# zhouhuan2005/deep-fusion

Measured on AMD Instinct MI355X. Metric: fused conv3x3+relu+conv1x1 int8 images/sec, higher is better.
Workload: dtype u8*s8->s32 (int8 MFMA), f32 requant, s32 out

## Files before the change

deep-fusion_amd/csrc/conv_mfma.cuh:

```cuda
#pragma once

#include <type_traits>

#include "dfx_device.cuh"

namespace dfx {

constexpr int MFMA_THREADS = 1024;
constexpr int MFMA_TEAMS = 2;
constexpr int MFMA_CW = 7;
constexpr int MFMA_NB = 4;
#ifndef DFX_STAMPS
constexpr int MFMA_CTRL_BYTES = 128;
#else
constexpr int MFMA_CTRL_BYTES = 128 + 16 * 8 * 4;
#endif
constexpr int MFMA_LC = 22;
constexpr int MFMA_SPIN_LIMIT = 1 << 24;

constexpr int MAGIC0_BITS = 0x4B400000;
constexpr float MAGIC0_F = 12582912.0f;
constexpr int MAGIC1_BITS = 0x3E22F983;
constexpr int MAGIC1_LO = -0x22F983;
constexpr int MAGIC1_HI = 0x7FFFFF - 0x22F983;

__host__ __device__ constexpr int mfma_cst_floats(int oc, int oc1) { return oc1 ? 3 * oc + 5 * oc1 : 5 * oc; }

constexpr int CTL_NEXT = 0;
constexpr int CTL_END = 1;
constexpr int CTL_FULL = 4;
constexpr int CTL_DONE = 8;
constexpr int CTL_INFO = 16;

__device__ __forceinline__ v16i mfma_i8(v4i a, v4i b, v16i c) {
  return __builtin_amdgcn_mfma_i32_32x32x32_i8(a, b, c, 0, 0, 0);
}

template <int CP>
__device__ __forceinline__ int chunk_swizzle(int X) {
  if (CP == 2) return (X >> 3) & 1;
  if (CP == 4) return (X >> 2) & 3;
  return (X >> 1) & 7;
}

struct MfmaGeom {
  int th, tw;
  int uy, ux;
  int linear;
  int total_units;
  int row_chunks;
  int tile_chunks;
  unsigned row_magic;
  unsigned tw_magic;
  unsigned upi_magic, ux_magic;
  int ntu;
  unsigned ntu_magic;
  int claim_limit;
  int mode0, mode1;
  int s0_uniform;
  float s0_value;
  int tile_stride;
  int static_rounds;
  int pool;
  int lazy_queue;
  int half_from;
  int *queue;
#ifdef DFX_STAMPS
  unsigned long long *prof;
#endif
#ifdef DFX_TRACE
  int *trace;
#endif
};

#ifdef DFX_TRACE
#define DFX_TRACE_AT(code, v0, v1)                                                                      \
  do {                                                                                                  \
    if ((int)threadIdx.x == __builtin_amdgcn_readfirstlane((int)threadIdx.x)) {  \
      int *tr_ = g.trace + ((size_t)blockIdx.x * 16 + (threadIdx.x >> 6)) * 4;                          \
      __hip_atomic_fetch_add(tr_ + 3, 1, __ATOMIC_RELAXED, __HIP_MEMORY_SCOPE_SYSTEM);  \
      if ((threadIdx.x & 63) != 0 && tr_[1] == 0)    \
        __hip_atomic_store(tr_ + 1, (int)(code), __ATOMIC_RELAXED, __HIP_MEMORY_SCOPE_SYSTEM);           \
      (void)(v0);                                                                                       \
      __hip_atomic_store(tr_ + 2, (int)__builtin_amdgcn_read_exec_lo(), __ATOMIC_RELAXED, __HIP_MEMORY_SCOPE_SYSTEM); (void)(v1); \
      __hip_atomic_store(tr_ + 0, (int)(code), __ATOMIC_RELEASE, __HIP_MEMORY_SCOPE_SYSTEM);            \
    }                                                                                                   \
  } while (0)
#else
#define DFX_TRACE_AT(code, v0, v1)
#endif

#ifdef DFX_STAMPS
__device__ __forceinline__ unsigned long long dfx_stamp() {
  unsigned long long t;
  __builtin_amdgcn_sched_barrier(0);
  asm volatile("s_memtime %0\n\ts_waitcnt lgkmcnt(0)" : "=s"(t)::"memory");
  __builtin_amdgcn_sched_barrier(0);
  return t;
}
#define DFX_STAMP(var) const unsigned long long var = dfx_stamp()
#define DFX_ACC(slot, expr) prof_acc[slot] += (expr)
#define DFX_TLOG(n, v0, v1, v2, v3)                                                                      \
  do {                                                                                                   \
    if ((n) < 8) {                                                                                       \
      unsigned long long *tl_ = g.prof + (size_t)gridDim.x * 256 +                                       \
                                (((size_t)blockIdx.x * 16 + (threadIdx.x >> 6)) * 8 + (n)) * 4;          \
      tl_[0] = (v0); tl_[1] = (v1); tl_[2] = (v2); tl_[3] = (v3);                                        \
    }                                                                                                    \
  } while (0)
#define DFX_LACC(slot, expr)                                                                             \
  __hip_atomic_fetch_add(ctrl + 32 + 8 * (int)(threadIdx.x >> 6) + (slot), (int)(unsigned)(expr), __ATOMIC_RELAXED, \
                         __HIP_MEMORY_SCOPE_WORKGROUP)
#else
#define DFX_STAMP(var)
#define DFX_ACC(slot, expr)
#define DFX_LACC(slot, expr)
#define DFX_TLOG(n, v0, v1, v2, v3)
#endif
// ... 281 lines not shown
      hrow = (v & 1) * hth;
    }
    n = g.upi_magic ? (int)__umulhi((unsigned)unit, g.upi_magic) : unit;
    const int u = unit - n * upi;
    uyi = g.ux_magic ? (int)__umulhi((unsigned)u, g.ux_magic) : u;
    uxi = u - uyi * g.ux;
  };
  auto unit_origin = [&](int unit, const uint8_t *&src_n, int &y0, int &x0) {
    int n, uyi, uxi, hrow, hth;
    unit_split(unit, n, uyi, uxi, hrow, hth);
    y0 = uyi * g.th + hrow - a.pt;
    x0 = uxi * g.tw - a.pl;
    src_n = a.src + (size_t)n * a.ih * a.iw * IC;
  };

  auto unit_info = [&](int unit, int &pix0, int &thtw, int &tprm) {
    int n, uyi, uxi, hrow, hth;
    unit_split(unit, n, uyi, uxi, hrow, hth);
    const int y0 = uyi * g.th + hrow, x0 = uxi * g.tw;
    const int th = max(0, min(hth, a.oh - y0)), tw = min(g.tw, a.ow - x0);
    const int tpr = g.pool ? (tw + 15) >> 4 : (tw + 31) >> 5;
    pix0 = g.pool ? (n * (a.oh >> 1) + (y0 >> 1)) * (a.ow >> 1) + (x0 >> 1)
                  : (n * a.oh + y0) * a.ow + x0;
    thtw = (th << 16) | tw;
    tprm = tpr > 1 ? (int)(((1ull << 32) + tpr - 1) / tpr) : 0;
  };

  const int wg = (gridDim.x % 8 == 0) ? (int)(blockIdx.x % 8) * (int)(gridDim.x / 8) + (int)(blockIdx.x / 8)
                                      : (int)blockIdx.x;
  auto stream_id = [&](int tm) { return tm * (int)gridDim.x + wg; };
  const bool coop0 = g.static_rounds >= 1;

  auto ctl_load = [&](int idx) {
    return __builtin_amdgcn_readfirstlane(
        __hip_atomic_load(ctrl + idx, __ATOMIC_ACQUIRE, __HIP_MEMORY_SCOPE_WORKGROUP));
  };
  auto ctl_store = [&](int idx, int v) {
    __hip_atomic_store(ctrl + idx, v, __ATOMIC_RELEASE, __HIP_MEMORY_SCOPE_WORKGROUP);
  };

  auto stage_weights = [&]() {
    constexpr int NT = MFMA_TEAMS * MFMA_CW * 64;
    constexpr int TT = MFMA_CW * 64;
    const int ctid = (team * MFMA_CW + cw) * 64 + lane, tctid = cw * 64 + lane;
    const v4i *s = reinterpret_cast<const v4i *>(a.wei);
    v4i *d = reinterpret_cast<v4i *>(w0s);
    const int total = OCB * 9 * ICB * 64 + NCB * OCB * 64 + (mfma_cst_floats(OC, OC1) * 4 + 15) / 16;
    unsigned char *slot = tiles + (size_t)team * g.tile_stride;
    const int unit0 = stream_id(team);
    const bool tile0 = coop0 && unit0 < g.total_units;
    const uint8_t *src_n = a.src;
    int y0 = 0, x0 = 0;
    if (tile0) unit_origin(unit0, src_n, y0, x0);
    for (int base = 0; base < total; base += 4 * NT) {
      const int q0 = base + ctid, last = total - 1;
      const v4i t0 = s[min(q0 + 0 * NT, last)];
      const v4i t1 = s[min(q0 + 1 * NT, last)];
      const v4i t2 = s[min(q0 + 2 * NT, last)];
      const v4i t3 = s[min(q0 + 3 * NT, last)];
      v4i u0 = x80, u1 = x80, u2 = x80, u3 = x80;
      if (tile0 && base == 0) {
        u0 = load_granule(src_n, y0, x0, min(tctid + 0 * TT, g.tile_chunks - 1));
        u1 = load_granule(src_n, y0, x0, min(tctid + 1 * TT, g.tile_chunks - 1));
        u2 = load_granule(src_n, y0, x0, min(tctid + 2 * TT, g.tile_chunks - 1));
        u3 = load_granule(src_n, y0, x0, min(tctid + 3 * TT, g.tile_chunks - 1));
      }
      d[min(q0 + 0 * NT, last)] = t0;
      d[min(q0 + 1 * NT, last)] = t1;
      d[min(q0 + 2 * NT, last)] = t2;
      d[min(q0 + 3 * NT, last)] = t3;
      if (tile0 && base == 0) {
        if (tctid + 0 * TT < g.tile_chunks) *reinterpret_cast<v4i *>(slot + 16 * (tctid + 0 * TT)) = u0;
        if (tctid + 1 * TT < g.tile_chunks) *reinterpret_cast<v4i *>(slot + 16 * (tctid + 1 * TT)) = u1;
        if (tctid + 2 * TT < g.tile_chunks) *reinterpret_cast<v4i *>(slot + 16 * (tctid + 2 * TT)) = u2;
        if (tctid + 3 * TT < g.tile_chunks) *reinterpret_cast<v4i *>(slot + 16 * (tctid + 3 * TT)) = u3;
      }
    }
    if (tile0) {
      for (int base = 4 * TT; base < g.tile_chunks; base += 4 * TT) {
        const int q0 = base + tctid;
        const v4i t0 = load_granule(src_n, y0, x0, min(q0 + 0 * TT, g.tile_chunks - 1));
        const v4i t1 = load_granule(src_n, y0, x0, min(q0 + 1 * TT, g.tile_chunks - 1));
        const v4i t2 = load_granule(src_n, y0, x0, min(q0 + 2 * TT, g.tile_chunks - 1));
        const v4i t3 = load_granule(src_n, y0, x0, min(q0 + 3 * TT, g.tile_chunks - 1));
        if (q0 + 0 * TT < g.tile_chunks) *reinterpret_cast<v4i *>(slot + 16 * (q0 + 0 * TT)) = t0;
        if (q0 + 1 * TT < g.tile_chunks) *reinterpret_cast<v4i *>(slot + 16 * (q0 + 1 * TT)) = t1;
        if (q0 + 2 * TT < g.tile_chunks) *reinterpret_cast<v4i *>(slot + 16 * (q0 + 2 * TT)) = t2;
        if (q0 + 3 * TT < g.tile_chunks) *reinterpret_cast<v4i *>(slot + 16 * (q0 + 3 * TT)) = t3;
      }
    }
    if (ctid < MFMA_CTRL_BYTES / 4) {
      int v = 0;
      if (ctid == CTL_END || ctid == CTL_END + 1) {
        v = 0x7fffffff;
        if (coop0 && stream_id(ctid - CTL_END) >= g.total_units) v = ctid - CTL_END;
      }
      auto first_unit = [&](int sl) {
        const int u = (sl >> 1) * (int)gridDim.x * MFMA_TEAMS + stream_id(sl & 1);
        return sl < 2 && coop0 && u < g.total_units ? u : -1;
      };
      if (ctid >= CTL_FULL && ctid < CTL_FULL + MFMA_NB && first_unit(ctid - CTL_FULL) >= 0) v = 1;
      if (ctid >= CTL_INFO && ctid < CTL_INFO + 4 * MFMA_NB) {
        const int u0 = first_unit((ctid - CTL_INFO) >> 2);
        if (u0 >= 0) {
          int i0, i1, i2;
          unit_info(u0, i0, i1, i2);
          const int f = (ctid - CTL_INFO) & 3;
          v = f == 0 ? i0 : f == 1 ? i1 : f == 2 ? i2 : 0;
        }
      }
      ctrl[ctid] = v;
    }
  };

  if (cw == MFMA_CW) {
#ifndef DFX_NO_SETPRIO
    __builtin_amdgcn_s_setprio(3);
#endif
    v4i pf[MFMA_LC];
    static_assert(MFMA_LC % 2 == 0, "rel table packs two entries per register");
    unsigned relp[MFMA_LC / 2];
#pragma unroll
    for (int i = 0; i < MFMA_LC; ++i) {
      const int q = min(lane + 64 * i, g.tile_chunks - 1);
      const int lr = (int)__umulhi((unsigned)q, g.row_magic);
      const int c = q - lr * g.row_chunks;
      const int X = c / CP;
      const unsigned r16 = (unsigned)((lr * a.iw + X) * CP + ((c % CP) ^ chunk_swizzle<CP>(X)));
      if (i % 2 == 0) relp[i / 2] = r16 & 0xffffu;
      else relp[i / 2] |= r16 << 16;
    }
    const int pad_half = (g.th + 2) * CP;
    int padoff[2], padside[2];
#pragma unroll
    for (int m = 0; m < 2; ++m) {
      const int e = lane + 64 * m, side = e >= pad_half ? 1 : 0, r = e - side * pad_half;
      padside[m] = e < 2 * pad_half ? side : 2;
      padoff[m] = (((r / CP) * LW + (side ? LW - 1 : 0)) * CP + (r % CP)) * 16;
    }
    const bool fast_ok = 2 * pad_half <= 128 && (g.th + 2) * a.iw * CP < 65536;
    auto unit_fast = [&](int unit, const uint8_t *&base_u, int &left, int &right) {
      const uint8_t *src_n;
      int y0, x0;
      unit_origin(unit, src_n, y0, x0);
      base_u = src_n + ((long long)y0 * a.iw + x0) * IC;
      left = x0 < 0;
      right = x0 + LW - 1 >= a.iw;
      return fast_ok && y0 >= 1 && y0 + g.th + 1 <= a.ih - 2 && x0 >= -1 && x0 + LW - 1 <= a.iw;
    };
    int cur_fast = 0, cur_left = 0, cur_right = 0;
#define DFX_PREFETCH(UNIT)                                                              \
  do {                                                                                  \
    const uint8_t *base_u_;                                                             \
    cur_fast = unit_fast((UNIT), base_u_, cur_left, cur_right) ? 1 : 0;                 \
    if (cur_fast) {                                                                     \
       \
      _Pragma("unroll") for (int i = 0; i < MFMA_LC; ++i) {                             \
        unsigned rp_ = relp[i / 2];  \
        asm volatile("" : "+v"(rp_));                                                   \
        pf[i] = *reinterpret_cast<const v4i *>(base_u_ + ((i % 2 ? rp_ >> 16 : rp_ & 0xffffu) << 4)); \
      }                                                                                 \
    } else {                                                                            \
      const uint8_t *src_n_;                                                            \
      int y0_, x0_;                                                                     \
      unit_origin((UNIT), src_n_, y0_, x0_);                                            \
      int lq_ = lane;  \
      asm volatile("" : "+v"(lq_));                                                     \
      _Pragma("unroll") for (int i = 0; i < MFMA_LC; ++i)                               \
          pf[i] = load_granule(src_n_, y0_, x0_, min(lq_ + 64 * i, g.tile_chunks - 1)) ^ x80; \
    }                                                                                   \
  } while (0)
    const int T = (int)gridDim.x * MFMA_TEAMS, tg = stream_id(team);
    const bool use_queue = g.static_rounds * T < g.total_units;
    auto unit_at = [&](int j) {
      int v = j * T + tg;
      if (j >= g.static_rounds) {
        v = 0x7fffffff;
        if (use_queue && lane == 0) v = g.static_rounds * T + atomicAdd(g.queue, 1);
      }
      return v;
    };

    auto write_tile = [&](unsigned char *ins) {
      {
        unsigned char *dst = ins + lane * 16;
        const int dump = g.tile_stride - 1024;
#pragma unroll
        for (int i = 0; i < MFMA_LC; ++i)
          *reinterpret_cast<v4i *>(dst + (64 * i < g.tile_chunks ? 1024 * i : dump)) = pf[i] ^ x80;
      }
      if (cur_fast) {
#pragma unroll
        for (int m = 0; m < 2; ++m)
          if ((padside[m] == 0 && cur_left) || (padside[m] == 1 && cur_right))
            *reinterpret_cast<v4i *>(ins + padoff[m]) = x80;
      }
    };
    auto write_rest = [&](unsigned char *ins, int unit) {
      if (g.tile_chunks > 64 * MFMA_LC) {
        const uint8_t *src_n; int y0, x0;
        unit_origin(unit, src_n, y0, x0);
        for (int q = 64 * MFMA_LC + lane; q < g.tile_chunks; q += 64)
          *reinterpret_cast<v4i *>(ins + 16 * q) = load_granule(src_n, y0, x0, q);
      }
    };
    DFX_STAMP(l_pre);
    const int j0 = coop0 ? 1 : 0;
    if (coop0) __syncthreads();
    const bool lazy = use_queue && g.lazy_queue;
    int cur = lazy ? 0 : __builtin_amdgcn_readfirstlane(unit_at(j0));
    int nxt_v = lazy ? 0 : unit_at(j0 + 1);
    int jn = j0 + 2;
    if (!lazy && cur < g.total_units) DFX_PREFETCH(cur);
    if (!coop0) __syncthreads();
    DFX_STAMP(l_post);
#ifdef DFX_STAMPS
    if (lane == 0) {
      unsigned long long *o = g.prof + ((size_t)blockIdx.x * 16 + wave) * 16;
      o[13] = l_pre - t_entry;
      o[14] = l_post - l_pre;
    }
#endif

    DFX_TRACE_AT(100, cur, j0);
    for (int j = j0;; ++j) {
      DFX_STAMP(la);
      const int s = 2 * (j & 1) + team, gen = j >> 1;
      DFX_TRACE_AT(101, cur, j);
      unsigned char *ins = tiles + (size_t)s * g.tile_stride;
      if (lazy) {
        for (int spin = 0; spin < MFMA_SPIN_LIMIT && ctl_load(CTL_DONE + s) < 64 * g.ntu * gen; ++spin)
          __builtin_amdgcn_s_sleep(8);
        cur = __builtin_amdgcn_readfirstlane(unit_at(j));
        if (cur < g.total_units) DFX_PREFETCH(cur);
      }
      const bool valid = cur < g.total_units;
      if (!valid) {
        if (!(coop0 && j == 1 && tg >= g.total_units)) ctl_store(CTL_END + team, 2 * j + team);
        break;
      }
      for (int spin = 0; spin < MFMA_SPIN_LIMIT && ctl_load(CTL_DONE + s) < 64 * g.ntu * gen; ++spin)
        __builtin_amdgcn_s_sleep(2);
      DFX_STAMP(lb);
      write_tile(ins);
      write_rest(ins, cur);
      DFX_TRACE_AT(102, cur, j);
      {
        int i0, i1, i2;
        unit_info(cur, i0, i1, i2);
        ctrl[CTL_INFO + 4 * s + 0] = i0;
        ctrl[CTL_INFO + 4 * s + 1] = i1;
        ctrl[CTL_INFO + 4 * s + 2] = i2;
      }
      __builtin_amdgcn_fence(__ATOMIC_RELEASE, "workgroup");
      ctl_store(CTL_FULL + s, gen + 1);
      DFX_STAMP(lc);
      if (!lazy) {
        cur = __builtin_amdgcn_readfirstlane(nxt_v);
        nxt_v = unit_at(jn++);
        if (cur < g.total_units) DFX_PREFETCH(cur);
      }
      DFX_STAMP(ld);
#ifdef DFX_STAMPS
      DFX_LACC(0, lb - la); DFX_LACC(1, lc - lb); DFX_LACC(2, ld - lc); DFX_LACC(3, 1);
      DFX_TLOG(j - j0, la - t_entry, lb - t_entry, lc - t_entry, ((unsigned long long)(ld - t_entry) << 16) | (unsigned)(2 * j + team));
#endif
    }
#ifdef DFX_STAMPS
    if (lane == 0) {
      unsigned long long *o = g.prof + ((size_t)blockIdx.x * 16 + wave) * 16;
      for (int k = 0; k < 4; ++k) o[k] = (unsigned)ctrl[32 + 8 * wave + k] / 64u;
    }
#endif
#undef DFX_PREFETCH
    DFX_TRACE_AT(103, cur, 0);
    const int pending = __builtin_amdgcn_readfirstlane(nxt_v);
    if (use_queue && lane == 0 && pending >= 0) {
      const int fin = atomicAdd(g.queue + 1, 1);
      if (fin == (int)gridDim.x * MFMA_TEAMS - 1) {
        atomicExch(g.queue, 0);
        atomicExch(g.queue + 1, 0);
      }
    }
    DFX_TRACE_AT(199, 0, 0);
    return;
  }

  DFX_TRACE_AT(1, 0, 0);
  stage_weights();
  DFX_TRACE_AT(2, 0, 0);
  DFX_STAMP(t_staged);
  __syncthreads();
  const int *ia0 = reinterpret_cast<const int *>(cst);
  const float *fb0 = cst + OC, *fc0 = cst + 2 * OC;
  const v2f *pb0 = reinterpret_cast<const v2f *>(cst + OC), *pc0 = reinterpret_cast<const v2f *>(cst + 3 * OC);
  const int *ia1 = reinterpret_cast<const int *>(cst + 3 * OC);
  const v2f *pb1 = reinterpret_cast<const v2f *>(cst + 3 * OC + OC1), *pc1 = reinterpret_cast<const v2f *>(cst + 3 * OC + 3 * OC1);
  const bool relu1 = (FUSED ? a.relu1 : a.relu0) || DST == DFX_U8;
  const int mode0 = g.mode0, mode1 = g.mode1;
  const unsigned row_bytes = (unsigned)(FUSED ? OC1 : OC) * ESZ;
  const int lds_row = LW * IC;

  DFX_STAMP(t_loop);
#ifdef DFX_STAMPS
  int tl_n = 0;
#endif
  DFX_LACC(4, t_loop - t_entry);
#ifdef DFX_STAMPS
  const unsigned long long startup_stage = t_staged - t_entry;
#endif
  DFX_TRACE_AT(3, 0, 0);
  typedef __attribute__((address_space(3))) int lds_int;
  auto draw = [&]() { return __builtin_amdgcn_ds_append((lds_int *)(ctrl + CTL_NEXT)); };
  struct Look { int full, end; v4i info; };
  auto look = [&](int sl, int par) {
    Look l;
    l.full = __hip_atomic_load(ctrl + CTL_FULL + sl, __ATOMIC_ACQUIRE, __HIP_MEMORY_SCOPE_WORKGROUP);
    l.info[0] = __hip_atomic_load(ctrl + CTL_INFO + 4 * sl + 0, __ATOMIC_RELAXED, __HIP_MEMORY_SCOPE_WORKGROUP);
    l.info[1] = __hip_atomic_load(ctrl + CTL_INFO + 4 * sl + 1, __ATOMIC_RELAXED, __HIP_MEMORY_SCOPE_WORKGROUP);
    l.info[2] = __hip_atomic_load(ctrl + CTL_INFO + 4 * sl + 2, __ATOMIC_RELAXED, __HIP_MEMORY_SCOPE_WORKGROUP);
    l.info[3] = 0;
    l.end = __hip_atomic_load(ctrl + CTL_END + par, __ATOMIC_RELAXED, __HIP_MEMORY_SCOPE_WORKGROUP);
    return l;
  };
  auto split = [&](int t, int &k, int &ti) {
    k = g.ntu == 1 ? t : (int)__umulhi((unsigned)t, g.ntu_magic);
    ti = t - k * g.ntu;
  };
  int c_ahead = 0;
  int t = __builtin_amdgcn_readfirstlane(draw()) >> 6, k, ti;
  split(t, k, ti);
  Look lk = look(k & (MFMA_NB - 1), k & 1);
  for (;;) {
    DFX_STAMP(c0);
// ... 357 lines not shown
```

deep-fusion_amd/csrc/conv_mfma_roles.cuh:

```cuda
#pragma once

#include "conv_mfma.cuh"

namespace dfx {

#ifndef RL_RING
#define RL_RING 5
#endif
#ifndef RL_NA
#define RL_NA 6
#endif
#ifndef RL_NB
#define RL_NB 8
#endif
constexpr int RL_A = RL_NA;
constexpr int RL_B = RL_NB;
constexpr int RL_C = RL_A + RL_B;
constexpr int RL_WAVES = RL_C + MFMA_TEAMS;
constexpr int RL_THREADS = 64 * RL_WAVES;
constexpr int RL_CTRL_BYTES = 512;
constexpr int MAGIC3_BITS = 0x4B000000;
constexpr int RL_SPIN_LIMIT = 1 << 19;

constexpr int RCTL_ADONE = 33;
// ... 117 lines not shown
    static_assert(MFMA_LC % 2 == 0, "rel table packs two entries per register");
    unsigned relp[MFMA_LC / 2];
#pragma unroll
    for (int i = 0; i < MFMA_LC; ++i) {
      const int q = min(lane + 64 * i, g.tile_chunks - 1);
      const int lr = (int)__umulhi((unsigned)q, g.row_magic);
      const int c = q - lr * g.row_chunks;
      const int X = c / CP;
      const unsigned r16 = (unsigned)((lr * a.iw + X) * CP + ((c % CP) ^ chunk_swizzle<CP>(X)));
      if (i % 2 == 0) relp[i / 2] = r16 & 0xffffu;
      else relp[i / 2] |= r16 << 16;
    }
    const int pad_half = (g.th + 2) * CP;
    int padoff[2], padside[2];
#pragma unroll
    for (int m = 0; m < 2; ++m) {
      const int e = lane + 64 * m, side = e >= pad_half ? 1 : 0, r = e - side * pad_half;
      padside[m] = e < 2 * pad_half ? side : 2;
      padoff[m] = (((r / CP) * LW + (side ? LW - 1 : 0)) * CP + (r % CP)) * 16;
    }
    const bool fast_ok = 2 * pad_half <= 128 && (g.th + 2) * a.iw * CP < 65536;
    auto unit_fast = [&](int unit, const uint8_t *&base_u, int &left, int &right) {
      const uint8_t *src_n;
      int y0, x0;
      unit_origin(unit, src_n, y0, x0);
      base_u = src_n + ((long long)y0 * a.iw + x0) * IC;
      left = x0 < 0;
      right = x0 + LW - 1 >= a.iw;
      return fast_ok && y0 >= 1 && y0 + g.th + 1 <= a.ih - 2 && x0 >= -1 && x0 + LW - 1 <= a.iw;
    };
    int cur_fast = 0, cur_left = 0, cur_right = 0;
#define DFX_PREFETCH(UNIT)                                                              \
  do {                                                                                  \
    const uint8_t *base_u_;                                                             \
    cur_fast = unit_fast((UNIT), base_u_, cur_left, cur_right) ? 1 : 0;                 \
    if (cur_fast) {                                                                     \
      _Pragma("unroll") for (int i = 0; i < MFMA_LC; ++i) {                             \
        unsigned rp_ = relp[i / 2];                                                     \
        asm volatile("" : "+v"(rp_));                                                   \
        pf[i] = *reinterpret_cast<const v4i *>(base_u_ + ((i % 2 ? rp_ >> 16 : rp_ & 0xffffu) << 4)); \
      }                                                                                 \
    } else {                                                                            \
      const uint8_t *src_n_;                                                            \
      int y0_, x0_;                                                                     \
      unit_origin((UNIT), src_n_, y0_, x0_);                                            \
      int lq_ = lane;                                                                   \
      asm volatile("" : "+v"(lq_));                                                     \
      _Pragma("unroll") for (int i = 0; i < MFMA_LC; ++i)                               \
          pf[i] = load_granule(src_n_, y0_, x0_, min(lq_ + 64 * i, g.tile_chunks - 1)) ^ x80; \
    }                                                                                   \
  } while (0)
    const int T = (int)gridDim.x * MFMA_TEAMS, tg = stream_id(team);
    const bool use_queue = g.static_rounds * T < g.total_units;
    auto unit_at = [&](int j) {
      int v = j * T + tg;
      if (j >= g.static_rounds) {
        v = 0x7fffffff;
        if (use_queue && lane == 0) v = g.static_rounds * T + atomicAdd(g.queue, 1);
      }
      return v;
    };
    auto write_tile = [&](unsigned char *ins) {
      {
        unsigned char *dst = ins + lane * 16;
        const int dump = g.tile_stride - 1024;
#pragma unroll
        for (int i = 0; i < MFMA_LC; ++i)
          *reinterpret_cast<v4i *>(dst + (64 * i < g.tile_chunks ? 1024 * i : dump)) = pf[i] ^ x80;
      }
      if (cur_fast) {
#pragma unroll
        for (int m = 0; m < 2; ++m)
          if ((padside[m] == 0 && cur_left) || (padside[m] == 1 && cur_right))
            *reinterpret_cast<v4i *>(ins + padoff[m]) = x80;
      }
    };
    auto write_rest = [&](unsigned char *ins, int unit) {
      if (g.tile_chunks > 64 * MFMA_LC) {
        const uint8_t *src_n; int y0, x0;
        unit_origin(unit, src_n, y0, x0);
        for (int q = 64 * MFMA_LC + lane; q < g.tile_chunks; q += 64)
          *reinterpret_cast<v4i *>(ins + 16 * q) = load_granule(src_n, y0, x0, q);
      }
    };
    const int j0 = coop0 ? 1 : 0;
    RL_ADD(8, dfx_stamp() - t_entry);
    if (coop0) __syncthreads();
    RL_ADD(9, dfx_stamp() - t_entry);
    const bool lazy = use_queue && g.lazy_queue;
    int cur = lazy ? 0 : __builtin_amdgcn_readfirstlane(unit_at(j0));
    int nxt_v = lazy ? 0 : unit_at(j0 + 1);
    int jn = j0 + 2;
    if (!lazy && cur < g.total_units) DFX_PREFETCH(cur);
    if (!coop0) __syncthreads();

    RL_ADD(4, dfx_stamp() - t_entry);
    for (int j = j0;; ++j) {
      DFX_STAMP(la);
      const int s = 2 * (j & 1) + team, gen = j >> 1;
      unsigned char *ins = tiles + (size_t)s * g.tile_stride;
      if (lazy) {
        for (int spin = 0; spin < MFMA_SPIN_LIMIT && ctl_load(CTL_DONE + s) < 64 * g.ntu * gen; ++spin)
          __builtin_amdgcn_s_sleep(8);
        cur = __builtin_amdgcn_readfirstlane(unit_at(j));
        if (cur < g.total_units) DFX_PREFETCH(cur);
      }
      const bool valid = cur < g.total_units;
      if (!valid) {
        if (!(coop0 && j == 1 && tg >= g.total_units)) ctl_store(CTL_END + team, 2 * j + team);
        break;
      }
      for (int spin = 0; spin < MFMA_SPIN_LIMIT && ctl_load(CTL_DONE + s) < 64 * g.ntu * gen; ++spin)
        __builtin_amdgcn_s_sleep(2);
      DFX_STAMP(lb);
      write_tile(ins);
      write_rest(ins, cur);
      {
        int i0, i1, i2;
        unit_info(cur, i0, i1, i2);
        ctrl[CTL_INFO + 4 * s + 0] = i0;
        ctrl[CTL_INFO + 4 * s + 1] = i1;
        ctrl[CTL_INFO + 4 * s + 2] = i2;
      }
      __builtin_amdgcn_fence(__ATOMIC_RELEASE, "workgroup");
      ctl_store(CTL_INFO + 4 * s + 3, gen + 1);
      DFX_STAMP(lc);
      if (!lazy) {
        cur = __builtin_amdgcn_readfirstlane(nxt_v);
        nxt_v = unit_at(jn++);
        if (cur < g.total_units) DFX_PREFETCH(cur);
      }
      DFX_STAMP(ld);
      RL_ADD(0, lb - la); RL_ADD(1, lc - lb); RL_ADD(2, ld - lc); RL_ADD(3, 1);
    }
#undef DFX_PREFETCH
    RL_FLUSH(2);
    const int pending = __builtin_amdgcn_readfirstlane(nxt_v);
    if (use_queue && lane == 0 && pending >= 0) {
      const int fin = atomicAdd(g.queue + 1, 1);
      if (fin == (int)gridDim.x * MFMA_TEAMS - 1) {
        atomicExch(g.queue, 0);
        atomicExch(g.queue + 1, 0);
      }
    }
    return;
  }

  {
    constexpr int CWT = RL_C / 2;
    constexpr int TT = CWT * 64;
    const int steam = wave / CWT, ctid = wave * 64 + lane, tctid = (wave % CWT) * 64 + lane;
    const v4i *s = reinterpret_cast<const v4i *>(a.wei);
    v4i *d = reinterpret_cast<v4i *>(w0s);
    const int total = OCB * 9 * ICB * 64 + NCB * OCB * 64 + (mfma_cst_floats(OC, OC1) * 4 + 15) / 16;
    unsigned char *slot = tiles + (size_t)steam * g.tile_stride;
    const int unit0 = stream_id(steam);
    const bool tile0 = coop0 && unit0 < g.total_units;
    const uint8_t *src_n = a.src;
    int y0 = 0, x0 = 0;
    if (tile0) unit_origin(unit0, src_n, y0, x0);
    {
      typedef __attribute__((address_space(3))) void lds_void;
      typedef __attribute__((address_space(1))) const void global_void;
      constexpr int w1_first = OCB * 9 * ICB * 64, w1_end = w1_first + NCB * OCB * 64;
      const int nblk = (total + 63) >> 6;
      for (int j = wave; j < nblk; j += RL_C) {
        const int q = 64 * j + lane;
        if (q < total && (q < w1_first || q >= w1_end))
          __builtin_amdgcn_global_load_lds((global_void *)(s + q), (lds_void *)(d + 64 * j), 16, 0, 0);
      }
      constexpr int NTL = 4;
      v4i tv[NTL];
      if (tile0) {
#pragma unroll
        for (int i = 0; i < NTL; ++i) tv[i] = load_granule(src_n, y0, x0, min(tctid + i * TT, g.tile_chunks - 1));
#pragma unroll
        for (int i = 0; i < NTL; ++i)
          if (tctid + i * TT < g.tile_chunks) *reinterpret_cast<v4i *>(slot + 16 * (tctid + i * TT)) = tv[i];
        for (int q = tctid + NTL * TT; q < g.tile_chunks; q += TT)
          *reinterpret_cast<v4i *>(slot + 16 * q) = load_granule(src_n, y0, x0, q);
      }
#ifdef DFX_STAMPS
      asm volatile("s_waitcnt vmcnt(0)" ::: "memory");
      RL_ADD(7, dfx_stamp() - t_entry);
#endif
    }
    if (ctid < RL_CTRL_BYTES / 4) {
      int v = 0;
      if (ctid == CTL_END || ctid == CTL_END + 1) {
        v = 0x7fffffff;
        if (coop0 && stream_id(ctid - CTL_END) >= g.total_units) v = ctid - CTL_END;
      }
      auto first_unit = [&](int sl) {
        const int u = (sl >> 1) * (int)gridDim.x * MFMA_TEAMS + stream_id(sl & 1);
        return sl < 2 && coop0 && u < g.total_units ? u : -1;
// ... 354 lines not shown
```

deep-fusion_amd/csrc/dfx_api.hip:

```cpp
#include <hip/hip_runtime.h>

#include <cstdarg>
#include <cstdio>
#include <algorithm>
#include <cmath>
#include <cstdlib>
#include <cstring>
#include <map>
#include <mutex>
#include <new>
#include <string>
#include <vector>

#include "conv_mfma.cuh"
#include "conv_stream.cuh"
#include "conv_direct.cuh"
#include "conv_pw.cuh"
#include "conv_mfma_roles.cuh"
#include "dfx_device.cuh"
#include "dfx_internal.h"

namespace dfx {
int launch_conv_generic(const ConvArgs &a, hipStream_t s, int *grid_out, int *lds_out);
#define DFX_DECL(n) \
  int launch_conv_mfma_##n(const ConvArgs &, const MfmaGeom &, int, int, int, int, int, hipStream_t, int)
DFX_DECL(f32);
DFX_DECL(s32);
DFX_DECL(s8);
DFX_DECL(u8);
#undef DFX_DECL
int launch_conv_mfma_roles_u8(const ConvArgs &, const MfmaGeom &, int, int, int, int, int, hipStream_t, int);
int launch_conv_mfma_roles_s8(const ConvArgs &, const MfmaGeom &, int, int, int, int, int, hipStream_t, int);
#define DFX_DECL(n) \
  int launch_conv_mfma_##n##_unfused(const ConvArgs &, const MfmaGeom &, int, int, int, int, hipStream_t, int)
DFX_DECL(f32);
DFX_DECL(s32);
DFX_DECL(s8);
DFX_DECL(u8);
#undef DFX_DECL

#define DFX_DECL(n) \
  int launch_conv_stream_##n(const ConvArgs &, const StreamGeom &, int, int, int, int, int, int, hipStream_t, int)
DFX_DECL(f32);
DFX_DECL(s32);
DFX_DECL(s8);
DFX_DECL(u8);
#undef DFX_DECL

#define DFX_DECL(n) \
  int launch_conv_direct_##n(const ConvArgs &, const DirectGeom &, int, int, int, int, int, int, hipStream_t, int)
DFX_DECL(f32);
DFX_DECL(s32);
DFX_DECL(s8);
DFX_DECL(u8);
#undef DFX_DECL

int launch_concat(const ConcatArgs &a, hipStream_t s);
int launch_pool(const PoolArgs &a, hipStream_t s);
int launch_eltwise(const EltwiseArgs &a, hipStream_t s);
}

using namespace dfx;

static thread_local char g_err[512] = "";

int dfx::fail(int code, const char *fmt, ...) {
  va_list ap;
  va_start(ap, fmt);
  vsnprintf(g_err, sizeof(g_err), fmt, ap);
  va_end(ap);
  return code;
}

namespace {
const char *const kTuningKeys[] = {"DFX_MAX_TH", "DFX_FORCE_GEOM", "DFX_STATIC_ROUNDS", "DFX_NO_FAST", "DFX_NO_MAGIC", "DFX_NO_LAZY", "DFX_HALF_UNITS", "DFX_NO_ROLES", "DFX_STORE_BOUND_BYTES",
                                   "DFX_STREAM_PXB", "DFX_STREAM_BLOCKING", "DFX_STREAM_PLANES", "DFX_STREAM_OCC_PAR",
                                   "DFX_STREAM_DIRECT", "DFX_STREAM_PW", "DFX_DIRECT_NPB", "DFX_DIRECT_NW", "DFX_DIRECT_WO1", "DFX_STREAM_GRID", "DFX_DEBUG_PTRS",
                                   "DEEPFUSION_PROFILE"};
struct Tuning {
  std::mutex mu;
  std::map<std::string, std::string> kv;
  Tuning() {
    for (const char *k : kTuningKeys)
      if (const char *v = getenv(k)) kv[k] = v;
  }
};
Tuning &tuning() {
  static Tuning t;
  return t;
}
const char *tune(const char *key) {
  static thread_local std::string held;
  Tuning &t = tuning();
  std::lock_guard<std::mutex> lk(t.mu);
  auto it = t.kv.find(key);
  if (it == t.kv.end()) return nullptr;
  held = it->second;
  return held.c_str();
}
struct StreamRegistry {
  std::mutex mu;
  std::map<hipStream_t, unsigned long long> live;
  unsigned long long next = 1;
};
StreamRegistry &streams() {
  static StreamRegistry r;
  return r;
}
unsigned long long stream_serial(hipStream_t st) {
  StreamRegistry &r = streams();
  std::lock_guard<std::mutex> lk(r.mu);
  auto it = r.live.find(st);
  return it == r.live.end() ? 0ull : it->second;
}
}

unsigned long long dfx::stream_serial_of(hipStream_t st) { return stream_serial(st); }

constexpr unsigned DFX_QUEUE_RING = 16;

struct dfx_conv {
  int device;
  dfx_conv_desc d;
  int variant;
  ConvArgs args;
  MfmaGeom geom;
  StreamGeom sgeom;
  DirectGeom dgeom;
// ... 740 lines not shown
      conv_release(h);
      return fail(DFX_ERR_HIP, "conv_create: cannot raise dynamic LDS limit to %d bytes", h->lds);
    }
    int per_cu = mfma_dispatch(h, h->args, h->geom, nullptr, 2);
    if (per_cu < 1) per_cu = 1;
    const int capacity = prop.multiProcessorCount * per_cu;
    h->sgeom.occ_par = (d.oc1x1 == 0 && h->sgeom.n_occ > 1 && h->sgeom.total_units < 2 * capacity) ? 1 : 0;
    if (const char *e = tune("DFX_STREAM_OCC_PAR")) h->sgeom.occ_par = (d.oc1x1 == 0 && h->sgeom.n_occ > 1 && atoi(e)) ? 1 : 0;
    if (h->sgeom.occ_par) {
      const int units = h->sgeom.total_units;
      if (!pick_stream_geometry(d, h->occ, h->G, h->pxb, true, h->sgeom, h->lds) || h->sgeom.total_units != units ||
          mfma_dispatch(h, h->args, h->geom, nullptr, 1) != 0) {
        conv_release(h);
        return fail(DFX_ERR_HIP, "conv_create: internal: chunk-parallel layout failed");
      }
      h->sgeom.occ_par = 1;
    }
    h->grid = std::min(h->sgeom.total_units * (h->sgeom.occ_par ? h->sgeom.n_occ : 1), capacity);
    if (const char *e = tune("DFX_STREAM_GRID")) h->grid = std::max(1, std::min(h->grid, atoi(e)));
#ifdef DFX_STAMPS
    if (hipMalloc((void **)&h->d_prof, (size_t)h->grid * 96 * 8) != hipSuccess ||
        hipMemset(h->d_prof, 0, (size_t)h->grid * 96 * 8) != hipSuccess) {
      conv_release(h);
      return fail(DFX_ERR_HIP, "conv_create: cannot allocate the stamp buffer");
    }
    h->sgeom.prof = h->d_prof;
#endif
    a.rows_per_unit = h->sgeom.thv;
    a.units_per_image = h->sgeom.uy * h->sgeom.ux;
    snprintf(h->kernel_name, sizeof(h->kernel_name), "conv_stream_kernel<%d,%d,%d,%d,%s%s>", h->occ, h->G, h->pxb,
             d.dst_dt, d.oc1x1 ? "fused" : "unfused", h->sgeom.occ_par ? ",occ_par" : "");
  } else if (d.fuse_pool && !(want_mfma && pick_geometry(d, h->geom, h->lds))) {
    conv_release(h);
    return fail(DFX_ERR_UNSUPPORTED, "conv_create: no unit geometry of the resident-weight kernel fits fused pooling here");
  } else if (want_mfma && pick_geometry(d, h->geom, h->lds, roles_eligible(d) ? RL_CTRL_BYTES : MFMA_CTRL_BYTES)) {
    const bool fused = d.oc1x1 > 0;
    h->roles_ok = roles_eligible(d);
    h->variant = fused ? DFX_VARIANT_MFMA_FUSED : DFX_VARIANT_MFMA_CONV;
    h->icb = d.ic / 32; h->ocb = d.oc / 32;
    const int ncb = d.oc1x1 / 32;
    h->G = fused ? ((ncb % 4 == 0) ? 4 : (ncb % 2 == 0 ? 2 : 1)) : h->ocb;
    {
      int dev = 0;
      hipDeviceProp_t prop;
      if (hipGetDevice(&dev) != hipSuccess || hipGetDeviceProperties(&prop, dev) != hipSuccess) {
        conv_release(h);
        return fail(DFX_ERR_HIP, "conv_create: cannot query the device");
      }
      h->grid = prop.multiProcessorCount;
      const int want = (h->geom.total_units + MFMA_TEAMS - 1) / MFMA_TEAMS;
      if (h->grid > want) h->grid = want;
    }
    h->block = MFMA_THREADS;
    if (hipMalloc((void **)&h->d_queue, 8 * DFX_QUEUE_RING) != hipSuccess ||
        hipMemset(h->d_queue, 0, 8 * DFX_QUEUE_RING) != hipSuccess) {
      conv_release(h);
      return fail(DFX_ERR_HIP, "conv_create: cannot allocate the unit queue");
    }
    h->geom.queue = h->d_queue;
    h->ring_mu = new (std::nothrow) std::mutex();
    if (!h->ring_mu) {
      conv_release(h);
      return fail(DFX_ERR_HIP, "out of host memory");
    }
    h->geom.mode0 = h->geom.mode1 = 0;
    {
      const int teams = h->grid * MFMA_TEAMS;
      const int rounds = (h->geom.total_units + teams - 1) / teams;
      h->geom.static_rounds = rounds <= 8 ? rounds : 3;
      const size_t out_px_bytes = (size_t)(d.oc1x1 > 0 ? d.oc1x1 : d.oc) * dt_size(d.dst_dt);
      h->geom.lazy_queue = 0;
      if (out_px_bytes >= store_bound_bytes() && rounds > 2 && !tune("DFX_NO_LAZY")) {
        h->geom.lazy_queue = 1;
        h->geom.static_rounds = 2;
      }
      if (const char *e = tune("DFX_STATIC_ROUNDS")) h->geom.static_rounds = std::min(rounds, std::max(0, atoi(e)));
      h->geom.half_from = 0x7fffffff;
      if (h->geom.lazy_queue && !h->geom.pool && h->geom.th % 2 == 0 && !h->roles_ok) {
        const int half_tiles = h->geom.linear ? ((h->geom.th / 2) * h->geom.tw + 31) / 32 : (h->geom.th / 2) * (h->geom.tw / 32);
        long long nh = half_tiles >= 7 ? 4LL * teams : 0;
        if (const char *e = tune("DFX_HALF_UNITS")) nh = std::max(0, atoi(e));
        nh = std::min<long long>(nh, (long long)h->geom.total_units - (long long)(h->geom.static_rounds + 1) * teams);
        if (nh > 0) {
          h->geom.half_from = h->geom.total_units - (int)nh;
          h->geom.total_units += (int)nh;
          h->geom.claim_limit =
              (int)std::min<long long>(0x7ffffff0LL, (long long)h->geom.ntu * ((long long)h->geom.total_units + 4));
        }
      }
    }
#ifdef DFX_STAMPS
    if (hipMalloc((void **)&h->d_prof, (size_t)h->grid * 768 * 8) != hipSuccess ||
        hipMemset(h->d_prof, 0, (size_t)h->grid * 768 * 8) != hipSuccess) {
      conv_release(h);
      return fail(DFX_ERR_HIP, "conv_create: cannot allocate the stamp buffer");
    }
    h->geom.prof = h->d_prof;
#endif
#ifdef DFX_TRACE
    {
      void *hp = nullptr, *dp = nullptr;
      if (hipHostMalloc(&hp, (size_t)h->grid * 16 * 4 * 4, hipHostMallocMapped) != hipSuccess ||
          hipHostGetDevicePointer(&dp, hp, 0) != hipSuccess) {
        conv_release(h);
        return fail(DFX_ERR_HIP, "conv_create: cannot allocate the trace buffer");
      }
      memset(hp, 0, (size_t)h->grid * 16 * 4 * 4);
      h->trace_host = (int *)hp;
      h->geom.trace = (int *)dp;
    }
#endif
    a.rows_per_unit = h->geom.th;
    a.units_per_image = h->geom.uy * h->geom.ux;
    snprintf(h->kernel_name, sizeof(h->kernel_name), "conv_mfma_fused_kernel<%d,%d,%d,%d%s>", h->icb,
             h->ocb, h->G, d.dst_dt, fused ? "" : ",unfused");
    if (mfma_dispatch(h, h->args, h->geom, nullptr, 1) != 0) {
      conv_release(h);
      return fail(DFX_ERR_HIP, "conv_create: cannot raise dynamic LDS limit to %d bytes", h->lds);
    }
  } else {
    h->variant = DFX_VARIANT_GENERIC;
    h->block = 256;
    launch_conv_generic(a, nullptr, &h->grid, &h->lds);
    a.rows_per_unit = 0;
    const bool big_dst = (long long)d.bs * d.oh * d.ow * (d.oc1x1 ? d.oc1x1 : d.oc) * (long long)dt_size(d.dst_dt) >= (1LL << 32) - 16;
    snprintf(h->kernel_name, sizeof(h->kernel_name), "conv_generic_kernel<dt=%d>%s", d.dst_dt,
             big_dst && d.force_variant != DFX_VARIANT_GENERIC ? " [dst >= 4 GiB: no MFMA kernel (32-bit dst offsets)]" : "");
  }
  *out = h;
  return DFX_OK;
}

static float bias_to_f32(const void *b, int dt, int c) {
  switch (dt) {
    case DFX_F32: return ((const float *)b)[c];
    case DFX_S32: return (float)((const int32_t *)b)[c];
    case DFX_S8: return (float)((const int8_t *)b)[c];
    case DFX_U8: return (float)((const uint8_t *)b)[c];
  }
  return 0.0f;
}
// ... 450 lines not shown
    HIP_TRY(hipMemcpy(h->d_consts, cst.data(), cst.size() * 4, hipMemcpyHostToDevice));
    h->args.wei = (const int8_t *)h->d_wei;
    h->args.wei1 = (const int8_t *)h->d_wei1;
    h->args.consts = (const float *)h->d_consts;
  }
  h->weights_set = true;
  return DFX_OK;
}

int dfx_conv_submit(dfx_conv_t *h, const void *src_dev, void *dst_dev, dfx_stream_t s) {
  if (!h || !src_dev || !dst_dev) return fail(DFX_ERR_INVALID, "conv_submit: null argument");
  if (!h->weights_set) return fail(DFX_ERR_STATE, "conv_submit: dfx_conv_set_weights not called");
  DeviceGuard dg(h->device);
  ConvArgs a = h->args;
  a.src = (const uint8_t *)src_dev;
  a.dst = dst_dev;
  MfmaGeom g = h->geom;
  if (g.queue) {
    const hipStream_t st = (hipStream_t)s;
    std::lock_guard<std::mutex> lk(*h->ring_mu);
    const unsigned slot = h->launch_seq++ % DFX_QUEUE_RING;
    if (h->launch_seq == 1) {
      h->first_stream = st;
      h->first_serial = stream_serial(st);
    }
    if (!h->multi_stream && st != h->first_stream) {
      h->multi_stream = true;
      hipEvent_t e0 = nullptr;
      HIP_TRY(hipEventCreateWithFlags(&e0, hipEventDisableTiming));
      const bool gone = h->first_serial != 0 && stream_serial(h->first_stream) != h->first_serial;
      hipError_t r = gone ? hipErrorContextIsDestroyed : hipEventRecord(e0, h->first_stream);
      if (r == hipSuccess) r = hipStreamWaitEvent(st, e0, 0);
      if (r == hipSuccess) {
        ++h->ring_waits;
        h->first_ev = e0;
        for (unsigned i = 0; i < DFX_QUEUE_RING; ++i)
          if (h->slot_state[i] == 1) {
            h->slot_state[i] = 2;
            h->slot_stream[i] = h->first_stream;
            h->slot_ev[i] = e0;
          }
      } else {
        (void)hipEventDestroy(e0);
        if (!gone) (void)hipGetLastError();
        HIP_TRY(hipDeviceSynchronize());
        for (unsigned i = 0; i < DFX_QUEUE_RING; ++i)
          if (h->slot_state[i] == 1) h->slot_state[i] = 0;
      }
    }
    if (h->slot_state[slot] == 2 && h->slot_stream[slot] != st) {
      HIP_TRY(hipStreamWaitEvent(st, h->slot_ev[slot], 0));
      ++h->ring_waits;
    }
    g.queue += 2 * slot;
    if (mfma_dispatch(h, a, g, st, 0) != 0) return fail(DFX_ERR_UNSUPPORTED, "conv_submit: no kernel instance for this op");
    HIP_TRY(hipGetLastError());
    h->slot_stream[slot] = st;
    h->slot_state[slot] = 1;
    if (h->multi_stream) {
      if (h->slot_ev[slot] == h->first_ev) h->slot_ev[slot] = nullptr;
      if (!h->slot_ev[slot]) HIP_TRY(hipEventCreateWithFlags(&h->slot_ev[slot], hipEventDisableTiming));
      HIP_TRY(hipEventRecord(h->slot_ev[slot], st));
      h->slot_state[slot] = 2;
    }
    return DFX_OK;
  }
  int rc;
  if (h->variant != DFX_VARIANT_GENERIC)
    rc = mfma_dispatch(h, a, g, (hipStream_t)s, 0);
  else
    rc = launch_conv_generic(a, (hipStream_t)s, nullptr, nullptr);
  if (rc != 0) return fail(DFX_ERR_UNSUPPORTED, "conv_submit: no kernel instance for this op");
  HIP_TRY(hipGetLastError());
  return DFX_OK;
}

static size_t conv_src_bytes(const dfx_conv_desc &d) { return (size_t)d.bs * d.ih * d.iw * d.ic; }
static size_t conv_dst_bytes(const dfx_conv_desc &d) {
  const size_t px = d.fuse_pool ? (size_t)(d.oh / 2) * (d.ow / 2) : (size_t)d.oh * d.ow;
  return (size_t)d.bs * px * (d.oc1x1 ? d.oc1x1 : d.oc) * dt_size(d.dst_dt);
}

int dfx_conv_submit_host(dfx_conv_t *h, const void *src_host, void *dst_host) {
  if (!h || !src_host || !dst_host) return fail(DFX_ERR_INVALID, "conv_submit_host: null argument");
  DeviceGuard dg(h->device);
  const size_t sb = conv_src_bytes(h->d), db = conv_dst_bytes(h->d);
  if (!h->d_src) {
    HIP_TRY(hipMalloc(&h->d_src, sb));
    HIP_TRY(hipMalloc(&h->d_dst, db));
    HIP_TRY(hipStreamCreateWithFlags(&h->host_stream, hipStreamNonBlocking));
  }
  HIP_TRY(hipMemcpyAsync(h->d_src, src_host, sb, hipMemcpyHostToDevice, h->host_stream));
  int rc = dfx_conv_submit(h, h->d_src, h->d_dst, h->host_stream);
  if (rc) return rc;
  HIP_TRY(hipMemcpyAsync(dst_host, h->d_dst, db, hipMemcpyDeviceToHost, h->host_stream));
  HIP_TRY(hipStreamSynchronize(h->host_stream));
  return DFX_OK;
}

int dfx_conv_query(const dfx_conv_t *h, dfx_conv_info *info) {
  if (!h || !info) return fail(DFX_ERR_INVALID, "conv_query: null argument");
  const dfx_conv_desc &d = h->d;
  memset(info, 0, sizeof(*info));
  info->variant = h->variant;
  info->grid = h->grid; info->block = h->block; info->lds_bytes = h->lds;
  info->rows_per_unit = h->args.rows_per_unit;
  info->device = h->device;
  const uint64_t px = (uint64_t)d.bs * d.oh * d.ow;
  const uint64_t mac = px * ((uint64_t)d.oc * d.ic * d.kh * d.kw + (uint64_t)d.oc1x1 * d.oc);
  info->algorithmic_ops = 2 * mac;
  info->algorithmic_bytes = conv_src_bytes(d) + conv_dst_bytes(d) +
                            (uint64_t)d.oc * d.ic * d.kh * d.kw + (uint64_t)d.oc1x1 * d.oc;
  snprintf(info->kernel_name, sizeof(info->kernel_name), "%s", h->kernel_name);
  return DFX_OK;
}

int dfx_debug_conv_sched(const dfx_conv_t *h, int32_t *out, int n) {
  if (!h || !out || n < 0) return fail(DFX_ERR_INVALID, "conv_sched: null argument");
  if (!h->geom.queue) return fail(DFX_ERR_UNSUPPORTED, "conv_sched: this op has no unit queue (%s)", h->kernel_name);
  const MfmaGeom &g = h->geom;
  int waits;
  {
    std::lock_guard<std::mutex> lk(*h->ring_mu);
    waits = h->ring_waits;
  }
  const int32_t v[13] = {g.th, g.tw, g.linear, g.uy, g.ux, g.total_units, g.half_from, g.static_rounds, g.lazy_queue,
                         g.pool, h->grid * MFMA_TEAMS, (h->roles_ok && h->roles) ? 1 : 0, waits};
  for (int i = 0; i < n && i < 13; ++i) out[i] = v[i];
  return DFX_OK;
}

#ifdef DK_DEBUG
int dfx_debug_read_bounds(dfx_conv_t *h, long long *out) {
  if (!h || !h->d_prof) return fail(DFX_ERR_STATE, "no debug buffer");
  HIP_TRY(hipMemcpy(out, h->d_prof, 64 * 8, hipMemcpyDeviceToHost));
  return DFX_OK;
}
#endif

#ifdef DFX_TRACE
int *dfx_debug_trace(dfx_conv_t *h) { return h ? h->trace_host : nullptr; }
#endif

#ifdef DFX_STAMPS
int dfx_debug_read_stamps(dfx_conv_t *h, unsigned long long *out, int max_entries) {
  if (!h || !h->d_prof) return fail(DFX_ERR_STATE, "no stamps");
  int n = h->grid * (h->variant == DFX_VARIANT_MFMA_STREAM ? (h->direct ? h->nw * 16 : 96) : 768);
  if (n > max_entries) n = max_entries;
  HIP_TRY(hipMemcpy(out, h->d_prof, (size_t)n * 8, hipMemcpyDeviceToHost));
  return n;
}
#endif

int dfx_conv_destroy(dfx_conv_t *h) {
  conv_release(h);
  return DFX_OK;
}

int dfx_debug_set_tuning(const char *key, const char *value) {
  if (!key) return fail(DFX_ERR_INVALID, "set_tuning: null key");
  bool known = false;
  for (const char *k : kTuningKeys) known = known || strcmp(k, key) == 0;
  if (!known) return fail(DFX_ERR_INVALID, "set_tuning: unknown switch %s", key);
  Tuning &t = tuning();
  std::lock_guard<std::mutex> lk(t.mu);
  if (value) t.kv[key] = value;
  else t.kv.erase(key);
  return DFX_OK;
}


int dfx_concat_create(const dfx_concat_desc *desc, dfx_concat_t **out) {
  if (!desc || !out || !desc->channels) return fail(DFX_ERR_INVALID, "concat_create: null argument");
  *out = nullptr;
  const dfx_concat_desc &d = *desc;
  if (d.n_inputs <= 0 || d.bs <= 0 || d.h <= 0 || d.w <= 0)
    return fail(DFX_ERR_INVALID, "concat: non-positive dimension");
  if (d.dt < DFX_F32 || d.dt > DFX_U8) return fail(DFX_ERR_INVALID, "concat: bad dtype");
  if (d.n_inputs > CONCAT_MAX_INPUTS)
    return fail(DFX_ERR_UNSUPPORTED, "concat: more than %d inputs", CONCAT_MAX_INPUTS);
  const int blk = dt_size(d.dt) == 1 ? 16 : 4;
// ... 200 lines not shown
```

Before: 1.649 million.

## Partition dynamic unit queue per XCD group with a shared remainder queue

Splits the dynamically claimed work units into eight per-XCD ranges, each with its own atomic counter on a separate cache line, plus a shared remainder queue used once a group's range runs dry. The goal is to cut cross-die atomic contention on one global counter and to keep neighbouring units (which share input halos) on the same XCD's L2. The queue buffer grows per ring slot and the finalizer resets every counter line. It also widens the weight-staging loop from four loads to five per iteration. In exchange, load balance between XCDs depends on the remainder share, and the code assumes blockIdx modulo 8 maps to an XCD.

```diff
diff --git a/deep-fusion_amd/csrc/conv_mfma.cuh b/deep-fusion_amd/csrc/conv_mfma.cuh
--- a/deep-fusion_amd/csrc/conv_mfma.cuh
+++ b/deep-fusion_amd/csrc/conv_mfma.cuh
@@ -2,6 +2,7 @@
 
 #include <type_traits>
 
+#include "conv_units.h"
 #include "dfx_device.cuh"
 
 namespace dfx {
@@ -64,6 +65,7 @@
   int pool;
   int lazy_queue;
   int half_from;
+  int xcd_units;
   int *queue;
 #ifdef DFX_STAMPS
   unsigned long long *prof;
@@ -451,12 +453,13 @@
     const uint8_t *src_n = a.src;
     int y0 = 0, x0 = 0;
     if (tile0) unit_origin(unit0, src_n, y0, x0);
-    for (int base = 0; base < total; base += 4 * NT) {
+    for (int base = 0; base < total; base += 5 * NT) {
       const int q0 = base + ctid, last = total - 1;
       const v4i t0 = s[min(q0 + 0 * NT, last)];
       const v4i t1 = s[min(q0 + 1 * NT, last)];
       const v4i t2 = s[min(q0 + 2 * NT, last)];
       const v4i t3 = s[min(q0 + 3 * NT, last)];
+      const v4i t4 = s[min(q0 + 4 * NT, last)];
       v4i u0 = x80, u1 = x80, u2 = x80, u3 = x80;
       if (tile0 && base == 0) {
         u0 = load_granule(src_n, y0, x0, min(tctid + 0 * TT, g.tile_chunks - 1));
@@ -468,6 +471,7 @@
       d[min(q0 + 1 * NT, last)] = t1;
       d[min(q0 + 2 * NT, last)] = t2;
       d[min(q0 + 3 * NT, last)] = t3;
+      d[min(q0 + 4 * NT, last)] = t4;
       if (tile0 && base == 0) {
         if (tctid + 0 * TT < g.tile_chunks) *reinterpret_cast<v4i *>(slot + 16 * (tctid + 0 * TT)) = u0;
         if (tctid + 1 * TT < g.tile_chunks) *reinterpret_cast<v4i *>(slot + 16 * (tctid + 1 * TT)) = u1;
@@ -571,11 +575,29 @@
   } while (0)
     const int T = (int)gridDim.x * MFMA_TEAMS, tg = stream_id(team);
     const bool use_queue = g.static_rounds * T < g.total_units;
+    const bool lazy = use_queue && g.lazy_queue;
+    const int xu = lazy ? g.xcd_units : 0;
     auto unit_at = [&](int j) {
       int v = j * T + tg;
       if (j >= g.static_rounds) {
-        v = 0x7fffffff;
-        if (use_queue && lane == 0) v = g.static_rounds * T + atomicAdd(g.queue, 1);
+        v = UNIT_NONE;
+        if (use_queue && lane == 0) v = unit_of_draw(g.total_units, g.static_rounds * T, xu, UNIT_REMAINDER, atomicAdd(g.queue, 1));
+      }
+      return v;
+    };
+    bool xdry = xu <= 0;
+    auto unit_lazy = [&](int j) {
+      if (j < g.static_rounds) return j * T + tg;
+      const int xg = (int)(blockIdx.x % UNIT_GROUPS);
+      int v = UNIT_NONE, d = 0;
+      if (!xdry) {
+        if (lane == 0) d = atomicAdd(g.queue + UNIT_QUEUE_LINE * (1 + xg), 1);
+        v = unit_of_draw(g.total_units, g.static_rounds * T, xu, xg, __builtin_amdgcn_readfirstlane(d));
+        xdry = v == UNIT_NONE;
+      }
+      if (xdry) {
+        if (lane == 0) d = atomicAdd(g.queue, 1);
+        v = unit_of_draw(g.total_units, g.static_rounds * T, xu, UNIT_REMAINDER, __builtin_amdgcn_readfirstlane(d));
       }
       return v;
     };
@@ -606,7 +628,6 @@
     DFX_STAMP(l_pre);
     const int j0 = coop0 ? 1 : 0;
     if (coop0) __syncthreads();
-    const bool lazy = use_queue && g.lazy_queue;
     int cur = lazy ? 0 : __builtin_amdgcn_readfirstlane(unit_at(j0));
     int nxt_v = lazy ? 0 : unit_at(j0 + 1);
     int jn = j0 + 2;
@@ -630,7 +651,7 @@
       if (lazy) {
         for (int spin = 0; spin < MFMA_SPIN_LIMIT && ctl_load(CTL_DONE + s) < 64 * g.ntu * gen; ++spin)
           __builtin_amdgcn_s_sleep(8);
-        cur = __builtin_amdgcn_readfirstlane(unit_at(j));
+        cur = unit_lazy(j);
         if (cur < g.total_units) DFX_PREFETCH(cur);
       }
       const bool valid = cur < g.total_units;
@@ -675,10 +696,9 @@
     DFX_TRACE_AT(103, cur, 0);
     const int pending = __builtin_amdgcn_readfirstlane(nxt_v);
     if (use_queue && lane == 0 && pending >= 0) {
-      const int fin = atomicAdd(g.queue + 1, 1);
+      const int fin = atomicAdd(g.queue + UNIT_QUEUE_FIN, 1);
       if (fin == (int)gridDim.x * MFMA_TEAMS - 1) {
-        atomicExch(g.queue, 0);
-        atomicExch(g.queue + 1, 0);
+        for (int c = 0; c <= UNIT_QUEUE_FIN; c += UNIT_QUEUE_LINE) atomicExch(g.queue + c, 0);
       }
     }
     DFX_TRACE_AT(199, 0, 0);
diff --git a/deep-fusion_amd/csrc/conv_mfma_roles.cuh b/deep-fusion_amd/csrc/conv_mfma_roles.cuh
--- a/deep-fusion_amd/csrc/conv_mfma_roles.cuh
+++ b/deep-fusion_amd/csrc/conv_mfma_roles.cuh
@@ -193,11 +193,29 @@
   } while (0)
     const int T = (int)gridDim.x * MFMA_TEAMS, tg = stream_id(team);
     const bool use_queue = g.static_rounds * T < g.total_units;
+    const bool lazy = use_queue && g.lazy_queue;
+    const int xu = lazy ? g.xcd_units : 0;
     auto unit_at = [&](int j) {
       int v = j * T + tg;
       if (j >= g.static_rounds) {
-        v = 0x7fffffff;
-        if (use_queue && lane == 0) v = g.static_rounds * T + atomicAdd(g.queue, 1);
+        v = UNIT_NONE;
+        if (use_queue && lane == 0) v = unit_of_draw(g.total_units, g.static_rounds * T, xu, UNIT_REMAINDER, atomicAdd(g.queue, 1));
+      }
+      return v;
+    };
+    bool xdry = xu <= 0;
+    auto unit_lazy = [&](int j) {
+      if (j < g.static_rounds) return j * T + tg;
+      const int xg = (int)(blockIdx.x % UNIT_GROUPS);
+      int v = UNIT_NONE, d = 0;
+      if (!xdry) {
+        if (lane == 0) d = atomicAdd(g.queue + UNIT_QUEUE_LINE * (1 + xg), 1);
+        v = unit_of_draw(g.total_units, g.static_rounds * T, xu, xg, __builtin_amdgcn_readfirstlane(d));
+        xdry = v == UNIT_NONE;
+      }
+      if (xdry) {
+        if (lane == 0) d = atomicAdd(g.queue, 1);
+        v = unit_of_draw(g.total_units, g.static_rounds * T, xu, UNIT_REMAINDER, __builtin_amdgcn_readfirstlane(d));
       }
       return v;
     };
@@ -228,7 +246,6 @@
     RL_ADD(8, dfx_stamp() - t_entry);
     if (coop0) __syncthreads();
     RL_ADD(9, dfx_stamp() - t_entry);
-    const bool lazy = use_queue && g.lazy_queue;
     int cur = lazy ? 0 : __builtin_amdgcn_readfirstlane(unit_at(j0));
     int nxt_v = lazy ? 0 : unit_at(j0 + 1);
     int jn = j0 + 2;
@@ -243,7 +260,7 @@
       if (lazy) {
         for (int spin = 0; spin < MFMA_SPIN_LIMIT && ctl_load(CTL_DONE + s) < 64 * g.ntu * gen; ++spin)
           __builtin_amdgcn_s_sleep(8);
-        cur = __builtin_amdgcn_readfirstlane(unit_at(j));
+        cur = unit_lazy(j);
         if (cur < g.total_units) DFX_PREFETCH(cur);
       }
       const bool valid = cur < g.total_units;
@@ -278,10 +295,9 @@
     RL_FLUSH(2);
     const int pending = __builtin_amdgcn_readfirstlane(nxt_v);
     if (use_queue && lane == 0 && pending >= 0) {
-      const int fin = atomicAdd(g.queue + 1, 1);
+      const int fin = atomicAdd(g.queue + UNIT_QUEUE_FIN, 1);
       if (fin == (int)gridDim.x * MFMA_TEAMS - 1) {
-        atomicExch(g.queue, 0);
-        atomicExch(g.queue + 1, 0);
+        for (int c = 0; c <= UNIT_QUEUE_FIN; c += UNIT_QUEUE_LINE) atomicExch(g.queue + c, 0);
       }
     }
     return;
diff --git a/deep-fusion_amd/csrc/conv_units.h b/deep-fusion_amd/csrc/conv_units.h
--- /dev/null
+++ b/deep-fusion_amd/csrc/conv_units.h
@@ -0,0 +1,33 @@
+#pragma once
+
+#if defined(__HIPCC__) || defined(__CUDACC__)
+#define DFX_UNITS_HD __host__ __device__
+#else
+#define DFX_UNITS_HD
+#endif
+
+namespace dfx {
+
+constexpr int UNIT_GROUPS = 8;
+constexpr int UNIT_REMAINDER = 8;
+constexpr int UNIT_NONE = 0x7fffffff;
+constexpr int UNIT_QUEUE_LINE = 32;
+constexpr int UNIT_QUEUE_FIN = UNIT_QUEUE_LINE * (1 + UNIT_GROUPS);
+constexpr int UNIT_QUEUE_SLOT_INTS = UNIT_QUEUE_LINE * (2 + UNIT_GROUPS);
+
+constexpr int UNIT_XCD_SHARE_PCT = 75;
+
+DFX_UNITS_HD inline int unit_xcd_range(int total_units, int half_from, int first, int share_pct, int workgroups) {
+  const int end = total_units < half_from ? total_units : half_from;
+  if (share_pct <= 0 || end <= first || workgroups <= 0 || workgroups % UNIT_GROUPS != 0) return 0;
+  const long long n = (long long)(end - first) * (share_pct < 100 ? share_pct : 100) / 100;
+  return (int)(n / UNIT_GROUPS);
+}
+
+DFX_UNITS_HD inline int unit_of_draw(int total_units, int first, int xcd_units, int group, int draw) {
+  if (group != UNIT_REMAINDER) return draw < xcd_units ? first + group * xcd_units + draw : UNIT_NONE;
+  const int base = first + UNIT_GROUPS * xcd_units;
+  return draw < total_units - base ? base + draw : UNIT_NONE;
+}
+
+}
diff --git a/deep-fusion_amd/csrc/dfx_api.hip b/deep-fusion_amd/csrc/dfx_api.hip
--- a/deep-fusion_amd/csrc/dfx_api.hip
+++ b/deep-fusion_amd/csrc/dfx_api.hip
@@ -73,7 +73,7 @@
 }
 
 namespace {
-const char *const kTuningKeys[] = {"DFX_MAX_TH", "DFX_FORCE_GEOM", "DFX_STATIC_ROUNDS", "DFX_NO_FAST", "DFX_NO_MAGIC", "DFX_NO_LAZY", "DFX_HALF_UNITS", "DFX_NO_ROLES", "DFX_STORE_BOUND_BYTES",
+const char *const kTuningKeys[] = {"DFX_MAX_TH", "DFX_FORCE_GEOM", "DFX_STATIC_ROUNDS", "DFX_NO_FAST", "DFX_NO_MAGIC", "DFX_NO_LAZY", "DFX_HALF_UNITS", "DFX_XCD_SHARE", "DFX_NO_ROLES", "DFX_STORE_BOUND_BYTES",
                                    "DFX_STREAM_PXB", "DFX_STREAM_BLOCKING", "DFX_STREAM_PLANES", "DFX_STREAM_OCC_PAR",
                                    "DFX_STREAM_DIRECT", "DFX_STREAM_PW", "DFX_DIRECT_NPB", "DFX_DIRECT_NW", "DFX_DIRECT_WO1", "DFX_STREAM_GRID", "DFX_DEBUG_PTRS",
                                    "DEEPFUSION_PROFILE"};
@@ -920,8 +920,8 @@
       if (h->grid > want) h->grid = want;
     }
     h->block = MFMA_THREADS;
-    if (hipMalloc((void **)&h->d_queue, 8 * DFX_QUEUE_RING) != hipSuccess ||
-        hipMemset(h->d_queue, 0, 8 * DFX_QUEUE_RING) != hipSuccess) {
+    if (hipMalloc((void **)&h->d_queue, sizeof(int) * UNIT_QUEUE_SLOT_INTS * DFX_QUEUE_RING) != hipSuccess ||
+        hipMemset(h->d_queue, 0, sizeof(int) * UNIT_QUEUE_SLOT_INTS * DFX_QUEUE_RING) != hipSuccess) {
       conv_release(h);
       return fail(DFX_ERR_HIP, "conv_create: cannot allocate the unit queue");
     }
@@ -955,6 +955,12 @@
           h->geom.claim_limit =
               (int)std::min<long long>(0x7ffffff0LL, (long long)h->geom.ntu * ((long long)h->geom.total_units + 4));
         }
+      }
+      h->geom.xcd_units = 0;
+      if (h->geom.lazy_queue) {
+        int share = UNIT_XCD_SHARE_PCT;
+        if (const char *e = tune("DFX_XCD_SHARE")) share = std::min(100, std::max(0, atoi(e)));
+        h->geom.xcd_units = unit_xcd_range(h->geom.total_units, h->geom.half_from, h->geom.static_rounds * teams, share, h->grid);
       }
     }
 #ifdef DFX_STAMPS
@@ -1511,7 +1517,7 @@
       HIP_TRY(hipStreamWaitEvent(st, h->slot_ev[slot], 0));
       ++h->ring_waits;
     }
-    g.queue += 2 * slot;
+    g.queue += UNIT_QUEUE_SLOT_INTS * slot;
     if (mfma_dispatch(h, a, g, st, 0) != 0) return fail(DFX_ERR_UNSUPPORTED, "conv_submit: no kernel instance for this op");
     HIP_TRY(hipGetLastError());
     h->slot_stream[slot] = st;
@@ -1586,6 +1592,7 @@
   const int32_t v[13] = {g.th, g.tw, g.linear, g.uy, g.ux, g.total_units, g.half_from, g.static_rounds, g.lazy_queue,
                          g.pool, h->grid * MFMA_TEAMS, (h->roles_ok && h->roles) ? 1 : 0, waits};
   for (int i = 0; i < n && i < 13; ++i) out[i] = v[i];
+  if (n > 13) out[13] = g.xcd_units;
   return DFX_OK;
 }
 
```

Result: slower. 1.625 million (-1.5%).
